# zhengchen1999/DOVE

Measured on AMD Instinct MI355X. Metric: SR frames/s (33x720x1280 4x one-step, whole job), higher is better.
Workload: dtype bf16; 1 GPU; synthetic 33x720x1280 HR clip (LR 180x320, 4x), one-step t=399, CogVideoX1.5-5B VAE + 42-layer DiT random-init, 1 clip per GPU (BASELINE configs[1]); weight_sums=True, vae_streams=2, variant=headline (bf16)

## Files before the change

dove_amd/csrc/igemm.hip:

```cpp
#include "igemm_args.h"


template <int BN, int BK>
struct FastCfg {
  static constexpr int BM = 128;
  static constexpr int CPR = BK / 8;
  static constexpr int CPR_LOG = (BK == 64) ? 3 : 2;
  static constexpr int RPG = 256 / CPR;
  static constexpr int NA = BM / RPG;
  static constexpr int B_SLOTS = BN * CPR;
  static constexpr int NB = (B_SLOTS + 255) / 256;
  static constexpr int A_BYTES = BM * BK * 2, B_BYTES = BN * BK * 2, STAGE = A_BYTES + B_BYTES;
  static constexpr int WN = (BN >= 128) ? 2 : 1, WM = 4 / WN;
  static constexpr int PT = (BM / WM) / 32, CT = (BN / WN) / 32;
  static constexpr int KK = BK / 16;
};

template <int BN, int BK>
__global__ __launch_bounds__(256) void igemm_fast_kernel(const IgemmArgs a) {
  using Cf = FastCfg<BN, BK>;
  constexpr int NA = Cf::NA, NB = Cf::NB, PT = Cf::PT, CT = Cf::CT, KK = Cf::KK, STAGE = Cf::STAGE, A_BYTES = Cf::A_BYTES;
  extern __shared__ __attribute__((aligned(16))) char smem[];
  const int tid = threadIdx.x, lane = tid & 63;
  const int wave = __builtin_amdgcn_readfirstlane(tid >> 6);
  __builtin_assume(wave >= 0 && wave < 4);
  const int wm = wave / Cf::WN, wn = wave % Cf::WN;

  unsigned rest = xcd_remap(blockIdx.x, gridDim.x);
  const int tn = rest % a.tiles_n; rest /= a.tiles_n;
  const int twi = rest % a.tiles_w; rest /= a.tiles_w;
  const int thi = rest % a.tiles_h;
  const int t = rest / a.tiles_h;
  const int n0 = tn * BN;
  const int TWm = (1 << a.tw_log2) - 1;
  const int oh0 = thi * (128 >> a.tw_log2), ow0 = twi << a.tw_log2;

  const int cs = tid & (Cf::CPR - 1);
  const int rsub = tid >> Cf::CPR_LOG;
  const int c = (BK == 64) ? (cs ^ ((rsub >> 1) & 7)) : (cs ^ ((rsub >> 2) & 3));
  int rowoff[NA];
  unsigned mask[NA];
#pragma unroll
  for (int j = 0; j < NA; ++j) {
    const int m = j * Cf::RPG + rsub;
    const int oh = oh0 + (m >> a.tw_log2), ow = ow0 + (m & TWm);
    const bool mv = (oh < a.H_out) && (ow < a.W_out);
    const int ih0 = oh * a.stride - a.pad_h, iw0 = ow * a.stride - a.pad_w;
    rowoff[j] = ((ih0 * a.W_in + iw0) * a.Cin + c * 8) * 2;
    unsigned mk = 0;
    for (int dh = 0; dh < a.kh; ++dh)
      for (int dw = 0; dw < a.kw; ++dw) {
        const bool ok = mv && ((unsigned)(ih0 + dh) < (unsigned)a.H_in) && ((unsigned)(iw0 + dw) < (unsigned)a.W_in);
        mk |= (ok ? 1u : 0u) << (dh * a.kw + dw);
      }
    mask[j] = mk;
  }
  int boff_g[NB];
#pragma unroll
  for (int j = 0; j < NB; ++j) boff_g[j] = ((j * Cf::RPG + rsub) * a.Cin + c * 8) * 2;

  const long long frame_elems = (long long)a.H_in * a.W_in * a.Cin;
  const unsigned frame_bytes = (unsigned)(frame_elems * 2);
  const unsigned wtap_bytes = (unsigned)((long long)BN * a.Cin * 2);
  const long long wtap_stride = (long long)a.Cout_pad * a.Cin;
  const int kc_per_tap = a.Cin / BK;
  const int nk = a.kt * a.kh * a.kw * kc_per_tap;

  auto frame_ptr = [&](int dt) -> const bf16_t* { return igemm_src_frame(a, t, dt, frame_elems); };
  int s_kc = 0, s_dw = 0, s_dh = 0, s_dt = 0;
  const bf16_t* s_fp = frame_ptr(0);
  const bf16_t* s_wp = a.w + (long long)n0 * a.Cin;
  int s_tapdelta = 0;
  unsigned s_tapbit = 1u;

  auto stage = [&](auto bufc) {
// ... 1037 lines not shown
  const bool pointwise = d->kt == 1 && d->kh == 1 && d->kw == 1 && d->stride == 1 && d->up == 0 && d->tmode == 0 && d->t_in == d->t_out &&
                         d->h_in == d->h_out && d->w_in == d->w_out;
  if (pointwise && d->cin == 32 && d->act == 0 && !d->resid && !d->gate && d->cout_store >= 128) return K_SMALLK;
  if (plain_gemm) {
    if (d->cout_pad % 256 == 0 && d->cout_store % 256 == 0 && d->cin % 128 == 0 && d->cin >= 256 && (long long)256 * d->cin * 2 < (1ll << 31) &&
        d->ldo < (1 << 20) && d->ldr < (1 << 20) && (d->act == 0 || d->act == 1))
      return K_GEMM8P;
  }
  const bool conv3 = d->kh == 3 && d->kw == 3 && d->stride == 1 && d->pad_h == 1 && d->pad_w == 1 && d->act == 0 && !d->gate &&
                     d->cout_pad % 128 == 0 && frame_fits;
  if (conv3) {
    const bool same = d->up == 0 && d->tmode == 0 && d->h_out == d->h_in && d->w_out == d->w_in && d->w_out >= 16 && d->h_out >= 16;
    const bool ups = d->up == 1 && d->kt == 1 && d->h_out == 2 * d->h_in && d->w_out == 2 * d->w_in && d->h_out >= 16 && d->w_out >= 32;
    const bool h4 = d->cout_store % 128 == 0 && d->cin % 64 == 0 && d->ldo < (1 << 20) && (!d->resid || d->ldr < (1 << 20));
    if (same && h4) return K_HALO4X;
    if (ups && h4 && d->w_sub && d->h_in >= 16 && d->w_in >= 32) return K_HALO4X_SUB;
    if (ups && h4) return K_HALO4X_UP;
  }
  const int BN = (d->cout_pad % 128 == 0) ? 128 : ((d->cout_pad % 64 == 0) ? 64 : 32);
  const bool fits = frame_fits && (long long)BN * d->cin * 2 < (1ll << 31);
  return (d->up == 0 && fits) ? K_IGEMM_FAST : K_IGEMM;
}

static bool desc_size_ok(const dove_conv_desc* d, const char* who) {
  if (d && d->struct_size == sizeof(dove_conv_desc) && d->reserved == 0) return true;
  if (d) dove_set_error("%s: dove_conv_desc.struct_size is %u, this library (ABI %d) expects %zu - the caller's binding was written "
                        "against another include/dove_hip.h", who, d->struct_size, DOVE_ABI_VERSION, sizeof(dove_conv_desc));
  else dove_set_error("%s: null descriptor", who);
  return false;
}
extern "C" const char* dove_conv_kernel_name(const dove_conv_desc* d) { return desc_size_ok(d, "conv_kernel_name") ? kKernelNames[select_kernel(d)] : ""; }

template <int BN, int BK>
static int launch_igemm_fast(const IgemmArgs& a, unsigned grid, hipStream_t s) {
  constexpr int lds = 2 * (128 * BK * 2 + BN * BK * 2);
  static PerDeviceOnce attr_set;
  if (auto once_ = attr_set.guard()) (void)hipFuncSetAttribute((const void*)igemm_fast_kernel<BN, BK>, hipFuncAttributeMaxDynamicSharedMemorySize, lds);
  hipLaunchKernelGGL((igemm_fast_kernel<BN, BK>), dim3(grid), dim3(256), lds, s, a);
  DOVE_CHECK_LAUNCH("dove_conv_igemm_bf16");
  return DOVE_OK;
}

static int cu_count() {
  static std::atomic<int> cus[DOVE_MAX_DEVICES] = {};
  int dev = 0;
  (void)hipGetDevice(&dev);
  int n = (dev >= 0 && dev < DOVE_MAX_DEVICES) ? cus[dev].load(std::memory_order_relaxed) : 0;
  if (!n) {
    n = 256;
    (void)hipDeviceGetAttribute(&n, hipDeviceAttributeMultiprocessorCount, dev);
    if (dev >= 0 && dev < DOVE_MAX_DEVICES) cus[dev].store(n, std::memory_order_relaxed);
  }
  return n;
}

extern "C" long long dove_conv_gn_partial_rows(const dove_conv_desc* d) {
  if (!desc_size_ok(d, "conv_gn_partial_rows")) return 0;
  const ConvKernel k = select_kernel(d);
  if (k != K_HALO4X && k != K_HALO4X_UP && k != K_HALO4X_SUB) return 0;
  if (d->cout_store != 128 && d->cout_store != 256 && d->cout_store != 512) return 0;
  if (d->cout_store != d->cout_pad) return 0;
  if (k == K_HALO4X_SUB) {
    const long long th = (d->h_in + halo8::TH - 1) / halo8::TH, tw = (d->w_in + halo8::TW - 1) / halo8::TW;
    return (long long)desc_nb(d) * d->t_out * th * tw * 16;
  }
  const long long th = (d->h_out + halo8::TH - 1) / halo8::TH, tw = (d->w_out + halo8::TW - 1) / halo8::TW;
  return (long long)desc_nb(d) * d->t_out * th * tw * 4;
}

static bool halo4x_plan(const dove_conv_desc* d) {
  const int tiles_w = (d->w_out + halo8::TW - 1) / halo8::TW, tiles_h = (d->h_out + halo8::TH - 1) / halo8::TH;
  const int wrem = d->w_out % halo8::TW;
  if (wrem < 1 || wrem > halo8::TW / 2) return false;
  const int cus = cu_count();
  const long long per = (long long)desc_nb(d) * d->t_out * (d->cout_pad / 128);
  auto rounds = [&](long long tiles) { return (tiles * per + cus - 1) / cus; };
  return rounds((long long)tiles_h * (tiles_w - 1)) + rounds((d->h_out + 31) / 32) < rounds((long long)tiles_h * tiles_w);
}
extern "C" int dove_conv_partial_launches(const dove_conv_desc* d) {
  if (!desc_size_ok(d, "conv_partial_launches") || select_kernel(d) != K_HALO4X) return 0;
  return halo4x_plan(d) ? 1 : 0;
}

static int conv_dispatch(const dove_conv_desc* d, void* stream, ConvKernel kern);

static bool gemm_tail_split(const dove_conv_desc* d, long long* rows_main) {
  const long long M = (long long)d->t_out * d->h_out * d->w_out;
  if (d->t_out != 1 || d->h_out != 1 || desc_nb(d) > 1) return false;
  const int cus = cu_count(), tiles_n = d->cout_pad / 256;
  const long long row_tiles = (M + gemm4x::BM - 1) / gemm4x::BM, ntiles = row_tiles * tiles_n;
  if (ntiles <= cus || ntiles % cus == 0) return false;
  const long long main_rt = (ntiles / cus) * cus / tiles_n;
  if (main_rt < 1 || main_rt >= row_tiles) return false;
  const long long tail_rows = M - main_rt * gemm4x::BM;
  const long long tail_blocks = ((tail_rows + 127) / 128) * (d->cout_pad / 128);
  if (tail_blocks > 2ll * cus) return false;
  if ((long long)128 * d->cin * 2 >= (1ll << 31)) return false;
  *rows_main = main_rt * gemm4x::BM;
  return true;
}

extern "C" int dove_conv_igemm_bf16(const dove_conv_desc* d, void* stream) {
  if (!desc_size_ok(d, "conv_igemm")) return DOVE_EINVAL;
  DOVE_CHECK_ARG(d->x && d->w && d->out, "conv_igemm: null pointer");
  DOVE_CHECK_ARG(d->cin % 32 == 0 && d->cin > 0, "conv_igemm: Cin (%d) must be a positive multiple of 32 (pad on pack)", d->cin);
  DOVE_CHECK_ARG(d->cout_pad % 32 == 0 && d->cout_pad > 0, "conv_igemm: Cout_pad (%d) must be a multiple of 32", d->cout_pad);
// ... 113 lines not shown
      a.cpg_log = d->cout_store == 128 ? 2 : (d->cout_store == 256 ? 3 : 4);
      a.tiles_w = (d->w_out + halo8::TW - 1) / halo8::TW;
      a.tiles_h = (d->h_out + halo8::TH - 1) / halo8::TH;
      a.tiles_n = d->cout_pad / 128;
      a.ty0 = a.tx0 = 0; a.nty = a.tiles_h; a.ntx = a.tiles_w; a.h_lim = d->h_out; a.w_lim = d->w_out;
      const long long g4 = (long long)a.T_out * a.tiles_h * a.tiles_w * a.tiles_n;
      DOVE_CHECK_ARG(g4 > 0 && g4 < (1ll << 31), "conv_igemm: grid too large");
      static PerDeviceOnce attr4;
      if (auto once_ = attr4.guard()) {
        (void)hipFuncSetAttribute((const void*)(conv3x3_halo4x_kernel<false>), hipFuncAttributeMaxDynamicSharedMemorySize, Halo4xCfg::LDS_BYTES);
        (void)hipFuncSetAttribute((const void*)(conv3x3_halo4x_kernel<false, false, 1>), hipFuncAttributeMaxDynamicSharedMemorySize, H4Geo<1>::LDS_BYTES);
        (void)hipFuncSetAttribute((const void*)(conv3x3_halo4x_kernel<true>), hipFuncAttributeMaxDynamicSharedMemorySize, Halo4xCfg::LDS_BYTES);
      }
      const int cus = cu_count();
      const unsigned grid = g4 > cus ? (unsigned)cus : (unsigned)g4;
      if (kern == K_HALO4X_UP) hipLaunchKernelGGL((conv3x3_halo4x_kernel<true>), dim3(grid), dim3(256), Halo4xCfg::LDS_BYTES, s, a);
      else {
        const bool wpart = halo4x_plan(d);
        const int wm = wpart ? (a.tiles_w - 1) * halo8::TW : d->w_out, cols_main = wpart ? a.tiles_w - 1 : a.tiles_w;
        auto launch = [&](int part, int nty, int tx0, int ntx, int w_lim) {
          if (nty <= 0 || ntx <= 0) return;
          IgemmArgs b = a;
          b.ty0 = 0; b.nty = nty; b.tx0 = tx0; b.ntx = ntx; b.h_lim = d->h_out; b.w_lim = w_lim;
          const long long g = (long long)b.T_out * nty * ntx * b.tiles_n;
          const unsigned gr = g > cus ? (unsigned)cus : (unsigned)g;
          if (part == 0) hipLaunchKernelGGL((conv3x3_halo4x_kernel<false, false, 0>), dim3(gr), dim3(256), H4Geo<0>::LDS_BYTES, s, b);
          else hipLaunchKernelGGL((conv3x3_halo4x_kernel<false, false, 1>), dim3(gr), dim3(256), H4Geo<1>::LDS_BYTES, s, b);
        };
        launch(0, a.tiles_h, 0, cols_main, wm);
        if (wpart) launch(1, (d->h_out + 31) / 32, cols_main, 1, d->w_out);
      }
      DOVE_CHECK_LAUNCH("dove_conv_igemm_bf16(halo4x)");
      return DOVE_OK;
    }
    default: break;
  }
  int twl = 7;
  if (d->h_out > 1) {
    twl = 4;
    if (d->w_out <= 8) twl = 3;
    if (d->w_out <= 4) twl = 2;
  }
  a.tw_log2 = twl;
  const int TW = 1 << twl, TH = 128 >> twl;
  a.tiles_w = (d->w_out + TW - 1) / TW;
  a.tiles_h = (d->h_out + TH - 1) / TH;
  const int BN = (d->cout_pad % 128 == 0) ? 128 : ((d->cout_pad % 64 == 0) ? 64 : 32);
  a.tiles_n = d->cout_pad / BN;
  const long long grid = (long long)a.T_out * a.tiles_h * a.tiles_w * a.tiles_n;
  DOVE_CHECK_ARG(grid > 0 && grid < (1ll << 31), "conv_igemm: grid too large");
  const bool fast = kern == K_IGEMM_FAST;
  const bool bk64 = (d->cin % 64 == 0);
  if (!fast) return launch_igemm_legacy(a, (unsigned)grid, BN, bk64, s);
  if (BN == 128) return bk64 ? launch_igemm_fast<128, 64>(a, (unsigned)grid, s) : launch_igemm_fast<128, 32>(a, (unsigned)grid, s);
  if (BN == 64) return bk64 ? launch_igemm_fast<64, 64>(a, (unsigned)grid, s) : launch_igemm_fast<64, 32>(a, (unsigned)grid, s);
  return bk64 ? launch_igemm_fast<32, 64>(a, (unsigned)grid, s) : launch_igemm_fast<32, 32>(a, (unsigned)grid, s);
}
```

dove_amd/lib.py:

```python
from __future__ import annotations

import ctypes as C
import os

import torch

_HERE = os.path.dirname(os.path.abspath(__file__))
LIB_PATH = os.path.join(_HERE, "libdove_hip.so")
_lib = None

F32, BF16, U8 = 0, 1, 2
METRIC_PSNR, METRIC_SSIM, METRIC_RGB_TO_Y = 1, 2, 4
COLORFIX_WAVELET, COLORFIX_ADAIN, COLORFIX_CLAMP = 1, 2, 1
YUV_444, YUV_422, YUV_420, YUV_MONO = 0, 1, 2, 3
YUV_SITING_LEFT, YUV_SITING_CENTRE = 0, 1
VIDEO_RGB_U8, VIDEO_YUV = 0, 1
RESIZE_BILINEAR, RESIZE_BICUBIC, RESIZE_AREA = 0, 1, 2
ACT_NONE, ACT_RELU, ACT_SIGMOID, ACT_TANH = 0, 1, 2, 3


class ConvDesc(C.Structure):
    _fields_ = [
        ("struct_size", C.c_uint), ("reserved", C.c_uint),
        ("x", C.c_void_p), ("cache", C.c_void_p), ("w", C.c_void_p), ("bias", C.c_void_p),
# ... 186 lines not shown
    "dove_vcodec_roundtrip_tools": [_VP, _I, _I, _I, _LL, _I, _I, _VP, C.c_size_t, _VP, _VP, _VP, _VP],
    "dove_motion_search_u8": [_VP, _VP, _I, _I, _I, _I, _I, _VP, _VP, _VP],
    "dove_stitch": [_VP, _I, _I, _I, _PI, _VP, _I, _I, _I, _I, _I, _I, _VP],
    "dove_video_open": [_VP, C.POINTER(VideoParams), C.POINTER(_VP)],
    "dove_video_info": [_VP, C.POINTER(C.c_size_t), C.POINTER(C.c_size_t), _PI, _PI, _PI],
    "dove_video_push": [_VP, _VP, _I, _VP],
    "dove_video_end_of_input": [_VP],
    "dove_video_need": [_VP, _PLL, _PI],
    "dove_video_step": [_VP, _VP, C.c_size_t, _PI, _PI, _VP],
    "dove_conv2d_f32": [C.POINTER(Conv2dF32Args), _VP],
    "dove_instance_norm_f32": [_VP, _I, _I, _I, _I, _VP, _I, _F, _VP, C.c_size_t, _VP, _VP],
    "dove_corr_volume_f32": [_VP, _VP, _I, _I, _I, _I, _F, _VP, _VP],
    "dove_avgpool2_f32": [_VP, _LL, _I, _I, _VP, _VP],
    "dove_corr_lookup_f32": [_VP, _VP, _VP, _VP, _VP, _LL, _I, _I, _I, _I, _VP, _VP],
    "dove_gru_gate_f32": [_VP, _LL, _VP, _LL, _I, _I, _LL, _VP, _VP],
    "dove_gru_update_f32": [_VP, _LL, _VP, _LL, _VP, _LL, _I, _LL, _VP],
    "dove_add_f32": [_VP, _LL, _VP, _LL, _VP, _LL, _I, _LL, _I, _VP],
    "dove_convex_upsample_f32": [_VP, _LL, _VP, _I, _I, _I, _VP, _VP],
    "dove_flow_warp_error": [_VP, _VP, _I, _VP, _VP, _I, _I, _I, _VP, C.c_size_t, _VP, _VP, _VP, _VP],
    "dove_convnet_conv_f32": [C.POINTER(ConvnetConvF32Args), _VP],
    "dove_percep_prep_f32": [C.POINTER(ImageView), _I, _I, _I, _I, _F, _F, C.POINTER(C.c_float), C.POINTER(C.c_float), _VP, _VP],
    "dove_maxpool_f32": [_VP, _LL, _I, _I, _I, _I, _I, _I, _VP, _LL, _VP],
    "dove_l2pool_f32": [_VP, _LL, _I, _I, _I, _I, _VP, _LL, _VP],
    "dove_lpips_layer": [_VP, _VP, _LL, _VP, _I, _I, _I, _I, _VP, C.c_size_t, _VP, _VP],
    "dove_dists_layer": [_VP, _VP, _LL, _VP, _VP, _I, _I, _I, _I, _VP, C.c_size_t, _VP, _VP],
    "dove_niqe_features": [C.POINTER(ImageView), _I, _I, _I, _I, _VP, C.c_size_t, _VP, _VP, _VP],
    "dove_niqe_stats": [_VP, _I, _I, _VP, _VP, _VP, _VP],
    "dove_niqe_distance": [_VP, _VP, _VP, _VP, _VP],
    "dove_resnet_conv_f32": [C.POINTER(ResnetConvF32Args), _VP],
    "dove_avgpool_cl_f32": [_VP, _LL, _I, _I, _I, _I, _VP, _LL, _VP],
    "dove_clip_attnpool_f32": [_VP, _LL, _I, _I, _I, _VP, _VP, _VP, _VP, _VP, _VP, _VP, _VP, _VP, C.c_size_t, _VP, _VP],
    "dove_clipiqa_score": [_VP, _VP, _I, _I, _I, C.c_double, _VP, _VP],
    "dove_musiq_patches_f32": [C.POINTER(ImageView), _I, _I, _I, _I, C.POINTER(MusiqScale), _VP, _I, _I, _I, _VP, _VP],
    "dove_musiq_groupnorm_f32": [_VP, _VP, _VP, _VP, _VP, _VP, _LL, _I, _I, C.c_double, _I, _I, _VP, _VP],
    "dove_layernorm_f32": [_VP, _LL, _LL, _I, _VP, _VP, C.c_double, _VP, _LL, _VP],
    "dove_musiq_embed_f32": [_VP, _VP, _VP, _VP, _VP, _I, _I, _I, _VP, _VP],
    "dove_mha_f32": [_VP, _VP, _VP, _LL, _I, _I, _I, _F, _VP, _LL, _VP],
    "dove_gelu_f32": [_VP, _LL, _VP, _VP],
    "dove_musiq_score": [_VP, _LL, _VP, _VP, _I, _I, _I, _VP, _VP],
    "dove_vqa_fragments_f32": [C.POINTER(ImageView), _I, _I, _I, _VP, _I, _VP, _I, _I, _I, _I, _I, C.POINTER(C.c_double), C.POINTER(C.c_double),
                               _I, _VP, _VP],
    "dove_swin3d_window_gather_f32": [_VP, _I, _PI, _I, _PI, _PI, _VP, _VP],
    "dove_swin3d_window_scatter_f32": [_VP, _VP, _I, _PI, _I, _PI, _PI, _VP, _VP],
    "dove_swin3d_patch_merge_f32": [_VP, _LL, _I, _I, _I, _VP, _VP],
    "dove_swin3d_window_attention_f32": [_VP, _VP, _VP, _LL, _LL, _I, _I, _F, _VP, _VP, _I, _VP, _VP, _VP, _I, _VP, _LL, _VP],
    "dove_vqa_head_f64": [_VP, _LL, _I, _I, _I, _VP, _VP, _I, _VP, _VP, _VP, _VP],
    "dove_png_encode": [C.POINTER(ImageView), _I, _I, _I, _I, _VP, C.c_size_t, _VP, _VP, _VP],
    "dove_zlib_huffman": [_VP, _LL, _LL, _VP, C.c_size_t, _VP, _VP, _VP],
}
PLAIN = {"dove_last_error": (C.c_char_p, []), "dove_abi_version": (C.c_int, []), "dove_comm_destroy": (None, [C.c_void_p]),
         "dove_conv_gn_partial_rows": (C.c_longlong, [C.POINTER(ConvDesc)]),
         "dove_conv_kernel_name": (C.c_char_p, [C.POINTER(ConvDesc)]),
         "dove_conv_partial_launches": (C.c_int, [C.POINTER(ConvDesc)]),
         "dove_attention_head_paths": (C.c_int, [C.POINTER(C.c_float), _I, C.POINTER(C.c_int)]),
         "dove_attention_path_name": (C.c_char_p, [_I]),
         "dove_device_info": (C.c_int, [_I, C.c_char_p, _I, C.POINTER(C.c_int), C.POINTER(C.c_longlong)]),
         "dove_destroy": (None, [_VP]),
         "dove_vae_decode_num_frames": (C.c_int, [_VP, _I]),
         "dove_get_option": (C.c_longlong, [_VP, _I]),
         "dove_comm_useful_ranks": (C.c_int, [_VP, _I, _I]),
         "dove_workspace_bytes": (C.c_size_t, [_VP, _I, _I, _I]),
         "dove_workspace_high_water": (C.c_size_t, [_VP]),
         "dove_fr_metrics_workspace_bytes": (C.c_size_t, [_I, _I, _I]),
         "dove_color_fix_workspace_bytes": (C.c_size_t, [_I, _I, _I, _I]),
         "dove_yuv_frame_bytes": (C.c_size_t, [_I, _I, _I]),
         "dove_poisson_noise_workspace_bytes": (C.c_size_t, [_I]),
         "dove_jpeg_roundtrip_workspace_bytes": (C.c_size_t, [_I, _I, _I]),
         "dove_vcodec_workspace_bytes": (C.c_size_t, [_I, _I, _I, _I]),
         "dove_vcodec_tools_workspace_bytes": (C.c_size_t, [_I, _I, _I, _I, _I]),
         "dove_chunk_planner_need": (C.c_longlong, [_VP]),
         "dove_chunk_planner_destroy": (None, [_VP]),
         "dove_video_workspace_bytes": (C.c_size_t, [_VP, C.POINTER(VideoParams)]),
         "dove_video_close": (None, [_VP]),
         "dove_instance_norm_f32_workspace_bytes": (C.c_size_t, [_I, _I, _I, _I]),
         "dove_flow_warp_error_workspace_bytes": (C.c_size_t, [_I, _I, _I]),
         "dove_convnet_conv_f32_kernel_name": (C.c_char_p, [C.POINTER(ConvnetConvF32Args)]),
         "dove_lpips_layer_workspace_bytes": (C.c_size_t, [_I, _I, _I]),
         "dove_dists_layer_workspace_bytes": (C.c_size_t, [_I, _I, _I, _I]),
         "dove_niqe_workspace_bytes": (C.c_size_t, [_I, _I, _I]),
         "dove_resnet_conv_f32_kernel_name": (C.c_char_p, [C.POINTER(ResnetConvF32Args)]),
         "dove_clip_attnpool_workspace_bytes": (C.c_size_t, [_I, _I, _I]),
         "dove_mha_f32_tiles": (None, [C.POINTER(C.c_int), C.POINTER(C.c_int)]),
         "dove_swin3d_attention_tiles": (None, [C.POINTER(C.c_int), C.POINTER(C.c_int), C.POINTER(C.c_int)]),
         "dove_png_segment_rows": (C.c_int, [_I, _I]),
         "dove_png_bound": (C.c_size_t, [_I, _I, _I]),
         "dove_png_workspace_bytes": (C.c_size_t, [_I, _I, _I, _I]),
         "dove_zlib_huffman_bound": (C.c_size_t, [_LL, _LL]),
         "dove_zlib_huffman_workspace_bytes": (C.c_size_t, [_LL, _LL])}


def kernel_source_sha256() -> str:
    import glob
    import hashlib
    h = hashlib.sha256()
    files = sorted(glob.glob(os.path.join(_HERE, "csrc", "*.hip")) + glob.glob(os.path.join(_HERE, "csrc", "*.h")))
    files.append(os.path.join(os.path.dirname(_HERE), "include", "dove_hip.h"))
    for fn in files:
        h.update(os.path.basename(fn).encode() + b"\0")
        with open(fn, "rb") as f:
            h.update(f.read())
        h.update(b"\0")
    return h.hexdigest()


def load():
    global _lib
# ... 53 lines not shown
```

dove_amd/ops.py:

```python
from __future__ import annotations

import ctypes as C
import math
from dataclasses import dataclass

import torch

from . import lib as L


def _ru(x: int, m: int) -> int:
    return (x + m - 1) // m * m


@dataclass
class PackedConv:
    w: torch.Tensor
    bias: torch.Tensor | None
    kt: int
    kh: int
    kw: int
    cin: int
    cin_pad: int
    cout: int
# ... 24 lines not shown
        bp[:cout] = bias.detach().to(device=device, dtype=torch.float32)
    wp = wp.contiguous()
    w_first = None
    if kt == 3:
        t = wp.float().view(3, kh * kw, cout_pad, cin_pad)
        s01 = t[0] + t[1]
        w_first = torch.stack([s01, s01 + t[2]]).to(torch.bfloat16).contiguous()
    w_pair = None
    if kt == 3 and pair:
        t = wp.float().view(3, kh * kw, cout_pad, cin_pad)
        w_pair = torch.stack([t[0] + t[1], t[1] + t[2]]).to(torch.bfloat16).contiguous()
    w_sub = None
    if kt == 1 and kh == 3 and kw == 3 and sub:
        t = wp.float().view(3, 3, cout_pad, cin_pad)
        w_sub = torch.zeros(4, 4, cout_pad, cin_pad, dtype=torch.float32, device=device)
        for py in range(2):
            for px in range(2):
                for dh in range(3):
                    for dw in range(3):
                        a, b = (py + dh + 1) // 2 - py, (px + dw + 1) // 2 - px
                        w_sub[2 * py + px, 2 * a + b] += t[dh, dw]
        w_sub = w_sub.to(torch.bfloat16).contiguous()
    return PackedConv(wp, bp, kt, kh, kw, cin, cin_pad, cout, cout_pad, w_first, w_sub, w_pair)


def temporal_split(tl: int, tdup: int, cached: bool, first_sums: bool = True):
    plain = [("w0", tl - 2), ("w1", tl - 1), ("w2", tl)]
    if tdup == 0:
        if cached or not first_sums or tl > 1:
            return plain
        return [("w012", 0)] if tl == 0 else [("w01", 0), ("w2", 1)]
    if tdup == 1:
        if not cached and tl < 2:
            return [("w012", tl)]
        return [("w0", tl - 2), ("w12", tl)] if tl & 1 else [("w01", tl - 1), ("w2", tl)]
    if tl == 0:
        return [("w012", 0)]
    return [("w01", tl - 1), ("w2", tl)] if tl & 1 else [("w0", tl - 2), ("w12", tl)]


def temporal_groups(tl: int, tdup: int, cached: bool) -> int:
    return len(temporal_split(tl, tdup, cached))


_profiler = None


def set_profiler(records: list | None):
    global _profiler
    _profiler = records


def conv_kernel_name(x_shape, pc: PackedConv, *, stride=1, pad=(None, None), up=0, tmode=0, t_out=None, hw_out=None, act=0, gated=False,
                     resid=False, nb=1, partial=False):
    T, H, W, Cx = x_shape
    d = L.ConvDesc()
    d.nb = nb
    ph = (pc.kh - 1) // 2 if pad[0] is None else pad[0]
    pw = (pc.kw - 1) // 2 if pad[1] is None else pad[1]
    t_out = T if t_out is None else t_out
    if hw_out is None:
        hw_out = (H << up, W << up) if stride == 1 else ((H + 1 - pc.kh) // stride + 1, (W + 1 - pc.kw) // stride + 1)
    d.t_in, d.h_in, d.w_in, d.cin = T, H, W, Cx
    d.t_out, d.h_out, d.w_out = t_out, hw_out[0], hw_out[1]
    d.cout_pad, d.cout_store = pc.cout_pad, pc.cout_store
    d.kt, d.kh, d.kw, d.stride, d.pad_h, d.pad_w = pc.kt, pc.kh, pc.kw, stride, ph, pw
    d.up, d.tmode, d.act = up, tmode, act
    d.ldo = pc.cout_store
    d.ldr = pc.cout_store if resid else 0
    d.resid = 1 if (resid or gated) else None
    d.w_sub = 1 if (up == 1 and pc.kt == 1 and pc.kh == 3 and pc.kw == 3) else None
    d.gate = 1 if gated else None
    if partial:
        return int(L.load().dove_conv_partial_launches(C.byref(d)))
    return L.load().dove_conv_kernel_name(C.byref(d)).decode()


def conv(x: torch.Tensor, pc: PackedConv, *, cache: torch.Tensor | None = None, stride: int = 1, pad=(None, None),
         up: int = 0, tmode: int = 0, t_out: int | None = None, hw_out=None, resid: torch.Tensor | None = None,
         gate: torch.Tensor | None = None, gate_split: int = 0, act: int = 0, ldo: int | None = None,
         out: torch.Tensor | None = None,
         gn_eps: float | None = None, out_f32: bool = False, nb: int = 1, tdup: int = 0, weight_sums: bool = True) -> torch.Tensor:
    L.require_cuda(x, resid, gate, out)
    assert x.dtype == torch.bfloat16 and x.dim() == 4, (x.dtype, x.shape)
    T, H, W, Cx = x.shape
    assert T % nb == 0, (T, nb)
    T //= nb
    if Cx != pc.cin_pad:
        raise RuntimeError(f"conv: input has {Cx} channels, packed weight expects {pc.cin_pad}")
    ph = (pc.kh - 1) // 2 if pad[0] is None else pad[0]
    pw = (pc.kw - 1) // 2 if pad[1] is None else pad[1]
    if t_out is None:
        t_out = T
    if hw_out is None:
        hw_out = (H << up, W << up) if stride == 1 else ((H + 1 - pc.kh) // stride + 1, (W + 1 - pc.kw) // stride + 1)
    if ldo is None:
        ldo = pc.cout_store
    odt = torch.float32 if out_f32 else torch.bfloat16
    if out is None:
        out = torch.empty(nb * t_out, hw_out[0], hw_out[1], ldo, dtype=odt, device=x.device)
    else:
        assert out.shape == (nb * t_out, hw_out[0], hw_out[1], ldo) and out.dtype == odt
    cache_stride = 0
    if cache is not None:
        if nb > 1:
            assert cache.shape == (nb, pc.kt - 1, H, W, Cx) and cache.dtype == torch.bfloat16 and cache.is_cuda, (cache.shape, x.shape)
            assert cache[0].is_contiguous() and cache.device == x.device
            cache_stride = cache.stride(0)
        else:
            L.require_cuda(cache)
            assert cache.shape == (pc.kt - 1, H, W, Cx) and cache.dtype == torch.bfloat16, (cache.shape, x.shape)
    d = L.ConvDesc()
    d.nb, d.cache_stride = nb, cache_stride
    if cache is None and pc.w_first is not None and weight_sums:
        d.w_first = pc.w_first.data_ptr()
    if up == 1 and pc.w_sub is not None and weight_sums:
        d.w_sub = pc.w_sub.data_ptr()
    if tdup and weight_sums and pc.w_pair is not None and pc.kt == 3 and not (tdup == 2 and cache is not None):
        d.tdup, d.w_pair = tdup, pc.w_pair.data_ptr()
    d.x, d.cache, d.w = x.data_ptr(), (cache.data_ptr() if cache is not None else None), pc.w.data_ptr()
    d.bias = pc.bias.data_ptr() if pc.bias is not None else None
    d.resid = resid.data_ptr() if resid is not None else None
    d.gate = gate.data_ptr() if gate is not None else None
    d.out = out.data_ptr()
    d.t_in, d.h_in, d.w_in, d.cin = T, H, W, Cx
    d.t_out, d.h_out, d.w_out = t_out, hw_out[0], hw_out[1]
    d.cout_pad, d.cout_store = pc.cout_pad, pc.cout_store
# ... 1353 lines not shown
```

include/dove_hip.h:

```cpp
#ifndef DOVE_HIP_H
#define DOVE_HIP_H

#include <stddef.h>

#ifdef __cplusplus
extern "C" {
#endif

#define DOVE_ABI_VERSION 15

#define DOVE_F32 0
#define DOVE_BF16 1

const char* dove_last_error(void);
int dove_abi_version(void);
int dove_device_info(int dev, char* name, int name_len, int* cu_count, long long* total_mem);

typedef struct dove_conv_desc {
  unsigned int struct_size;
  unsigned int reserved;
  const void* x;
  const void* cache;
  const void* w;
  const float* bias;
  const void* resid;
  const float* gate;
  void* out;
  int t_in, h_in, w_in, cin;
  int t_out, h_out, w_out, cout_pad, cout_store;
  int kt, kh, kw, stride, pad_h, pad_w, up, tmode, act;
  long long ldo, ldr, gate_split;
  float* gn_partial;
  int out_f32;
  int nb;
  long long cache_stride;
  const void* w_first;
  const void* w_sub;
  const void* w_pair;
  int tdup;
  int reserved2;
} dove_conv_desc;
int dove_conv_igemm_bf16(const dove_conv_desc* d, void* stream);
const char* dove_conv_kernel_name(const dove_conv_desc* d);
int dove_conv_partial_launches(const dove_conv_desc* d);
long long dove_conv_gn_partial_rows(const dove_conv_desc* d);
int dove_groupnorm_finalize_partials(const float* partial, long long rows, double count, float eps, void* ws, float* stats,
                                     void* stream);

int dove_groupnorm_stats_bf16(const void* x, long long npix, long long frame_pix, int C, float eps, void* partial_ws, int ws_blocks,
                              float* stats, void* stream);
int dove_groupnorm_sums_bf16(const void* x, long long npix, long long frame_pix, int C, void* partial_ws, int ws_blocks, double* sums,
                             void* stream);
int dove_groupnorm_finalize_sums(const double* sums, double count, float eps, float* stats, void* stream);
int dove_groupnorm_sums_from_partials(const float* partial, long long rows, void* ws, double* sums, void* stream);
int dove_groupnorm_apply_bf16(const void* x, void* y, int T, int H, int W, int C, const float* stats,
                              const float* gamma, const float* beta, int silu, const void* yb, int hz, int wz,
                              int sshift, const int* tmap, void* stream);

int dove_groupnorm_stats_nb_bf16(const void* x, int nb, long long npix, long long frame_pix, int C, float eps, void* partial_ws,
                                 int ws_blocks, float* stats, void* stream);
int dove_groupnorm_finalize_partials_nb(const float* partial, long long rows, int nb, double count, float eps, void* ws, size_t ws_bytes,
                                        float* stats, void* stream);
int dove_groupnorm_apply_nb_bf16(const void* x, void* y, int nb, int T, int H, int W, int C, const float* stats, const float* gamma,
                                 const float* beta, int silu, const void* yb, int Tz, int hz, int wz, int sshift, const int* tmap,
                                 void* stream);
int dove_avgpool_time_nb_bf16(const void* x, int nb, int T, long long frame_elems, void* y, void* stream);

int dove_layernorm_modulate_bf16(const void* x, void* y, long long rows, int D, float eps, const float* gamma,
                                 const float* beta, const float* mod, long long split, void* stream);

int dove_qkv_post_bf16(const void* qkv, long long N, long long Npad, int heads, int head_dim, int text_len,
                       const float* gq, const float* bq, const float* gk, const float* bk, const float* cosT,
                       const float* sinT, float qscale, float eps, void* Qh, void* Kh, void* Vt, int v_order, float* norm2, void* stream);
int dove_vt_quad_swap_bf16(void* Vt, long long rows, long long Npad, void* stream);
int dove_ulysses_place_bf16(const void* rq, const void* rk, const void* rv, const long long* counts, int world, int hloc, long long N,
                            long long Npad, void* Qh, void* Kh, void* Vt, float* norm2_out, void* stream);

int dove_attention_fwd_bf16(const void* Qh, const void* Kh, const void* Vt, void* O, long long N, long long Npad,
                            int heads, int head_dim, long long ldo, float* norm2, void* stream);
int dove_attention_head_paths(const float* norm2_host, int heads, int* path);
const char* dove_attention_path_name(int path);

int dove_cl_from_ncthw(const void* x, int dtype, int C, long long npix, int Cp, float scale, float shift, void* y,
                       void* stream);
int dove_ncthw_from_cl(const void* x, long long ld, int C, long long npix, float scale, float shift, float lo,
                       float hi, void* y, int dtype, void* stream);
int dove_cl_im2col3x3_from_ncthw(const void* x, int dtype, int C, int T, int H, int W, int Cp, float scale, float shift, void* y,
                                 void* stream);
int dove_conv_out_gather(const float* p, long long ldp, int T, int H, int W, int C, const float* bias, float scale, float shift, float lo,
                         float hi, void* y, int dtype, void* stream);
int dove_avgpool_time_bf16(const void* x, int T, long long frame_elems, void* y, void* stream);
int dove_posterior_sample(const void* moments, long long ld, int latent_channels, long long npix, const void* noise,
                          int noise_dtype, void* out, int out_dtype, void* stream);
int dove_axpby(const void* x, const void* y, void* out, int dtype, long long n, float a, float b, void* stream);
int dove_patchify(const void* x, int dtype, int T, int C, int H, int W, int pt, int p, void* tokens, long long ld,
                  void* stream);
int dove_unpatchify(const void* tokens, long long ld, int T, int C, int H, int W, int pt, int p, void* y, int dtype,
// ... 333 lines not shown
```

Measured before the change: 35.30 frames/s.

## Add persistent weight-resident streaming path for 1x1 igemm convolutions

Adds a persistent variant of the fast igemm kernel for 1x1 (optionally kt=3) convolutions with small K. Each workgroup loads its whole weight panel into LDS once, then walks a contiguous range of 128-row tiles. Activations stream through a 3- or 6-stage LDS ring of async buffer loads, and output stores overlap with later tiles via counted vmcnt waits. The grid is sized to CUs times waves per CU, which removes repeated weight loads and per-tile launch and prologue cost. The trade-off is hand-tuned wait counts and a larger LDS footprint, and the path only applies to plain 1x1 convs with no act, resid or gate.

```diff
diff --git a/dove_amd/csrc/igemm.hip b/dove_amd/csrc/igemm.hip
--- a/dove_amd/csrc/igemm.hip
+++ b/dove_amd/csrc/igemm.hip
@@ -16,11 +16,239 @@
   static constexpr int KK = BK / 16;
 };
 
-template <int BN, int BK>
+__device__ __forceinline__ const bf16_t* fs_pin64(const bf16_t* p) {
+  const unsigned long long v = (unsigned long long)p;
+  return (const bf16_t*)(((unsigned long long)(unsigned)__builtin_amdgcn_readfirstlane((int)(v >> 32)) << 32) |
+                         (unsigned)__builtin_amdgcn_readfirstlane((int)v));
+}
+typedef __attribute__((ext_vector_type(2))) unsigned int u32x2;
+template <int N> __device__ __forceinline__ void fs_wait_vm() {
+  asm volatile("s_waitcnt vmcnt(%0)" ::"n"(N < 63 ? N : 63) : "memory");
+}
+template <int BASE, int NST> __device__ __forceinline__ void fs_wait_counted(int cnt) {
+  if (cnt == 0) fs_wait_vm<BASE>();
+  else if (cnt == 1) fs_wait_vm<BASE + NST>();
+  else if (cnt == 2) fs_wait_vm<BASE + 2 * NST>();
+  else if (cnt == 3) fs_wait_vm<BASE + 3 * NST>();
+  else if (cnt == 4) fs_wait_vm<BASE + 4 * NST>();
+  else fs_wait_vm<BASE + 5 * NST>();
+}
+
+template <int BN, int BK, int NS>
+__device__ __forceinline__ void igemm_stream_walk(const IgemmArgs& a, char* smem) {
+  using Cf = FastCfg<BN, BK>;
+  constexpr int NA = Cf::NA, NB = Cf::NB, PT = Cf::PT, CT = Cf::CT, KK = Cf::KK, A_BYTES = Cf::A_BYTES, B_BYTES = Cf::B_BYTES;
+  constexpr int AHEAD = NS - 1;
+  constexpr int NST = PT * CT * 4;
+  constexpr int RING = NS * A_BYTES;
+  static_assert(NS >= 3 && NS <= 6, "ring of 3..6 stages (fs_wait_counted counts up to 5 epilogues)");
+  const int tid = threadIdx.x, lane = tid & 63;
+  const int wave = __builtin_amdgcn_readfirstlane(tid >> 6);
+  __builtin_assume(wave >= 0 && wave < 4);
+  const int wm = wave / Cf::WN, wn = wave % Cf::WN;
+  const int hi = lane >> 5, l31 = lane & 31;
+
+  const unsigned wg = xcd_remap(blockIdx.x, gridDim.x);
+  const int tn = (int)(wg % (unsigned)a.tiles_n), rb = (int)(wg / (unsigned)a.tiles_n), GR = (int)(gridDim.x / (unsigned)a.tiles_n);
+  const long long RT = (long long)a.T_out * a.tiles_h;
+  const int tile0 = __builtin_amdgcn_readfirstlane((int)(rb * RT / GR)), tile1 = __builtin_amdgcn_readfirstlane((int)((rb + 1) * RT / GR));
+  const int n0 = tn * BN;
+  const int HW = a.H_out * a.W_out;
+  const long long frame_elems = (long long)HW * a.Cin;
+  const unsigned frame_bytes = (unsigned)(frame_elems * 2);
+  const int kc_per_tap = a.Cin / BK;
+  const int nk = a.kt * kc_per_tap;
+  const int nsteps = (tile1 - tile0) * nk;
+
+  const int cs = tid & (Cf::CPR - 1);
+  const int rsub = tid >> Cf::CPR_LOG;
+  const int c = (BK == 64) ? (cs ^ ((rsub >> 1) & 7)) : (cs ^ ((rsub >> 2) & 3));
+  unsigned rowoff[NA];
+#pragma unroll
+  for (int j = 0; j < NA; ++j) rowoff[j] = (unsigned)(((j * Cf::RPG + rsub) * a.Cin + c * 8) * 2);
+
+  f32x4 biasr[CT][4];
+#pragma unroll
+  for (int i = 0; i < CT; ++i)
+#pragma unroll
+    for (int g = 0; g < 4; ++g) {
+      const int cb = n0 + wn * (BN / Cf::WN) + i * 32 + 8 * g + 4 * hi;
+      biasr[i][g] = (a.bias && cb < a.Cout_st) ? *(const f32x4*)(a.bias + cb) : f32x4{0.f, 0.f, 0.f, 0.f};
+    }
+  __builtin_amdgcn_s_waitcnt(0x0F70);
+
+  {
+    const unsigned wtap_bytes = (unsigned)((long long)BN * a.Cin * 2);
+    const bf16_t* wp = a.w + (long long)n0 * a.Cin;
+    int ks = 0;
+    for (int tap = 0; tap < a.kt; ++tap, wp += (long long)a.Cout_pad * a.Cin) {
+      const auto srd_b = __builtin_amdgcn_make_buffer_rsrc((void*)wp, (short)0, (int)wtap_bytes, 0x00020000);
+      for (int kc = 0; kc < kc_per_tap; ++kc, ++ks) {
+#pragma unroll
+        for (int j = 0; j < NB; ++j) {
+          if (j * 256 + wave * 64 < Cf::B_SLOTS)
+            __builtin_amdgcn_raw_ptr_buffer_load_lds(srd_b, (lds_ptr_t)(smem + RING + ks * B_BYTES + (j * 256 + wave * 64) * 16), 16,
+                                                     (unsigned)(((j * Cf::RPG + rsub) * a.Cin + c * 8) * 2), kc * (BK * 2), 0, 0);
+        }
+      }
+    }
+  }
+
+  int s_tile = tile0, s_t = tile0 / a.tiles_h, s_rt = tile0 - s_t * a.tiles_h, s_dt = 0, s_kc = 0;
+  const bf16_t* s_fp = a.x;
+  int s_nrec = 0;
+  auto open = [&]() {
+    const bool on = s_tile < tile1;
+    const long long roff = (long long)s_rt * 128 * a.Cin;
+    s_fp = fs_pin64(igemm_src_frame(a, on ? s_t : 0, s_dt, frame_elems) + roff);
+    s_nrec = on ? (int)(frame_bytes - (unsigned)(roff * 2)) : 0;
+  };
+  open();
+  auto stage = [&](int slot) {
+    const auto srd_a = __builtin_amdgcn_make_buffer_rsrc((void*)s_fp, (short)0, s_nrec, 0x00020000);
+    const int soff = s_kc * (BK * 2);
+#pragma unroll
+    for (int j = 0; j < NA; ++j)
+      __builtin_amdgcn_raw_ptr_buffer_load_lds(srd_a, (lds_ptr_t)(smem + slot * A_BYTES + (j * 256 + wave * 64) * 16), 16, rowoff[j], soff, 0, 0);
+    if (++s_kc == kc_per_tap) {
+      s_kc = 0;
+      if (++s_dt == a.kt) {
+        s_dt = 0;
+        ++s_tile;
+        if (++s_rt == a.tiles_h) { s_rt = 0; ++s_t; }
+      }
+      open();
+    }
+  };
+
+  int aoff[PT][KK], boff[CT][KK];
+#pragma unroll
+  for (int kk = 0; kk < KK; ++kk) {
+    const int chunk = kk * 2 + hi;
+#pragma unroll
+    for (int p = 0; p < PT; ++p) {
+      const int row = wm * (Cf::BM / Cf::WM) + p * 32 + l31;
+      const int sc = (BK == 64) ? (chunk ^ ((row >> 1) & 7)) : (chunk ^ ((row >> 2) & 3));
+      aoff[p][kk] = row * (BK * 2) + sc * 16;
+    }
+#pragma unroll
+    for (int i = 0; i < CT; ++i) {
+      const int row = wn * (BN / Cf::WN) + i * 32 + l31;
+      const int sc = (BK == 64) ? (chunk ^ ((row >> 1) & 7)) : (chunk ^ ((row >> 2) & 3));
+      boff[i][kk] = RING + row * (BK * 2) + sc * 16;
+    }
+  }
+
+  f32x16 acc[CT][PT];
+  auto zero_acc = [&]() {
+#pragma unroll
+    for (int i = 0; i < CT; ++i)
+#pragma unroll
+      for (int p = 0; p < PT; ++p)
+#pragma unroll
+        for (int r = 0; r < 16; ++r) acc[i][p][r] = 0.f;
+  };
+  zero_acc();
+
+  const int es = a.out_f32 ? 4 : 2;
+  const int ldo_b = (int)a.ldo * es;
+  unsigned ooff[PT];
+#pragma unroll
+  for (int p = 0; p < PT; ++p) ooff[p] = (unsigned)((wm * (Cf::BM / Cf::WM) + p * 32 + l31) * ldo_b);
+  auto epilogue = [&](int c_t, int c_rt, auto f32c, auto biasc) {
+    constexpr bool kF32 = decltype(f32c)::value, kBias = decltype(biasc)::value;
+    const int left = HW - c_rt * 128, rows = left < 128 ? left : 128;
+    const char* ob = (const char*)a.out + ((long long)c_t * HW + (long long)c_rt * 128) * ldo_b;
+    const auto srd_o = __builtin_amdgcn_make_buffer_rsrc((void*)fs_pin64((const bf16_t*)ob), (short)0, rows * ldo_b, 0x00020000);
+#pragma unroll
+    for (int p = 0; p < PT; ++p) {
+#pragma unroll
+      for (int i = 0; i < CT; ++i) {
+#pragma unroll
+        for (int g = 0; g < 4; ++g) {
+          const int cb = n0 + wn * (BN / Cf::WN) + i * 32 + 8 * g + 4 * hi;
+          float v[4];
+#pragma unroll
+          for (int e = 0; e < 4; ++e) v[e] = acc[i][p][g * 4 + e];
+          if (kBias) {
+#pragma unroll
+            for (int e = 0; e < 4; ++e) v[e] += biasr[i][g][e];
+          }
+          const unsigned voff = cb < a.Cout_st ? ooff[p] + (unsigned)(cb * es) : 0x80000000u;
+          if (kF32) {
+            __builtin_amdgcn_raw_buffer_store_b128(u32x4{__float_as_uint(v[0]), __float_as_uint(v[1]), __float_as_uint(v[2]), __float_as_uint(v[3])},
+                                                   srd_o, (int)voff, 0, 0);
+            __builtin_amdgcn_sched_barrier(0);
+            asm volatile("s_nop 3" ::: "memory");
+            __builtin_amdgcn_sched_barrier(0);
+          } else {
+            __builtin_amdgcn_raw_buffer_store_b64(u32x2{pack_bf2(v[0], v[1]), pack_bf2(v[2], v[3])}, srd_o, (int)voff, 0, 0);
+          }
+        }
+      }
+    }
+    __builtin_amdgcn_sched_barrier(0);
+    asm volatile("s_nop 3" ::: "memory");
+    __builtin_amdgcn_sched_barrier(0);
+  };
+
+#pragma unroll
+  for (int u = 0; u < AHEAD; ++u) stage(u);
+
+  int c_t = tile0 / a.tiles_h, c_rt = tile0 - c_t * a.tiles_h, c_k = 0;
+  int slot = 0, nslot = AHEAD;
+  unsigned hist = 0;
+  for (int s = 0; s < nsteps; ++s) {
+    fs_wait_counted<(AHEAD - 1) * NA, NST>(__builtin_popcount(hist & ((1u << AHEAD) - 1)));
+    __builtin_amdgcn_s_barrier();
+    asm volatile("" ::: "memory");
+    stage(nslot);
+    {
+      const int sa = slot * A_BYTES, sb = c_k * B_BYTES;
+#pragma unroll
+      for (int kk = 0; kk < KK; ++kk) {
+        bf16x8 xf[PT], wf[CT];
+#pragma unroll
+        for (int p = 0; p < PT; ++p) xf[p] = *(const bf16x8*)(smem + sa + aoff[p][kk]);
+#pragma unroll
+        for (int i = 0; i < CT; ++i) wf[i] = *(const bf16x8*)(smem + sb + boff[i][kk]);
+#pragma unroll
+        for (int i = 0; i < CT; ++i)
+#pragma unroll
+          for (int p = 0; p < PT; ++p)
+            acc[i][p] = __builtin_amdgcn_mfma_f32_32x32x16_bf16(wf[i], xf[p], acc[i][p], 0, 0, 0);
+      }
+    }
+    asm volatile("" ::: "memory");
+    slot = slot + 1 == NS ? 0 : slot + 1;
+    nslot = nslot + 1 == NS ? 0 : nslot + 1;
+    hist <<= 1;
+    if (++c_k == nk) {
+      if (a.out_f32) {
+        if (a.bias) epilogue(c_t, c_rt, std::true_type{}, std::true_type{});
+        else epilogue(c_t, c_rt, std::true_type{}, std::false_type{});
+      } else {
+        if (a.bias) epilogue(c_t, c_rt, std::false_type{}, std::true_type{});
+        else epilogue(c_t, c_rt, std::false_type{}, std::false_type{});
+      }
+      zero_acc();
+      c_k = 0;
+      hist |= 1u;
+      if (++c_rt == a.tiles_h) { c_rt = 0; ++c_t; }
+    }
+  }
+  asm volatile("s_waitcnt vmcnt(0)" ::: "memory");
+}
+
+template <int BN, int BK, int kStream = 0>
 __global__ __launch_bounds__(256) void igemm_fast_kernel(const IgemmArgs a) {
   using Cf = FastCfg<BN, BK>;
   constexpr int NA = Cf::NA, NB = Cf::NB, PT = Cf::PT, CT = Cf::CT, KK = Cf::KK, STAGE = Cf::STAGE, A_BYTES = Cf::A_BYTES;
   extern __shared__ __attribute__((aligned(16))) char smem[];
+  if constexpr (kStream > 0) {
+    igemm_stream_walk<BN, BK, kStream>(a, smem);
+    return;
+  }
   const int tid = threadIdx.x, lane = tid & 63;
   const int wave = __builtin_amdgcn_readfirstlane(tid >> 6);
   __builtin_assume(wave >= 0 && wave < 4);
@@ -1164,6 +1392,46 @@
     if (dev >= 0 && dev < DOVE_MAX_DEVICES) cus[dev].store(n, std::memory_order_relaxed);
   }
   return n;
+}
+
+struct StreamPlan { int ns, wpc; };
+static StreamPlan igemm_stream_plan(const dove_conv_desc* d) {
+  const StreamPlan no{0, 0};
+  if (select_kernel(d) != K_IGEMM_FAST) return no;
+  if (d->kh != 1 || d->kw != 1 || d->stride != 1 || d->up != 0 || d->nb > 1 || (d->kt != 1 && d->kt != 3)) return no;
+  if ((long long)d->kt * d->cin > 512) return no;
+  if (d->tmode != 0 || d->pad_h != 0 || d->pad_w != 0 || d->t_in != d->t_out || d->h_in != d->h_out || d->w_in != d->w_out) return no;
+  if (d->act != 0 || d->resid || d->gate || d->ldo >= (1 << 20)) return no;
+  const int BN = (d->cout_pad % 128 == 0) ? 128 : ((d->cout_pad % 64 == 0) ? 64 : 32), BK = (d->cin % 64 == 0) ? 64 : 32;
+  const int panel = d->kt * d->cin * BN * 2, stage = 128 * BK * 2, lds_cu = 160 * 1024;
+  StreamPlan p;
+  if (panel + 6 * stage <= lds_cu / 2) p = StreamPlan{6, 2};
+  else if (panel + 6 * stage <= lds_cu) p = StreamPlan{6, 1};
+  else if (panel + 3 * stage <= lds_cu) p = StreamPlan{3, 1};
+  else return no;
+  const long long row_tiles = (long long)d->t_out * (((long long)d->h_out * d->w_out + 127) / 128);
+  if (row_tiles < 2ll * cu_count() || row_tiles >= (1ll << 31)) return no;
+  return p;
+}
+extern "C" int dove_conv_igemm_fast_streams(const dove_conv_desc* d) {
+  if (!desc_size_ok(d, "conv_igemm_fast_streams")) return 0;
+  return igemm_stream_plan(d).ns ? 1 : 0;
+}
+
+template <int BN, int BK, int NS>
+static int launch_igemm_stream(const IgemmArgs& a, unsigned grid, hipStream_t s) {
+  const int lds = NS * (128 * BK * 2) + a.kt * a.Cin * BN * 2;
+  static PerDeviceOnce attr_set;
+  if (auto once_ = attr_set.guard()) (void)hipFuncSetAttribute((const void*)igemm_fast_kernel<BN, BK, NS>, hipFuncAttributeMaxDynamicSharedMemorySize, 160 * 1024);
+  hipLaunchKernelGGL((igemm_fast_kernel<BN, BK, NS>), dim3(grid), dim3(256), lds, s, a);
+  DOVE_CHECK_LAUNCH("dove_conv_igemm_bf16(stream)");
+  return DOVE_OK;
+}
+template <int NS>
+static int launch_igemm_stream_ns(const IgemmArgs& a, unsigned grid, int BN, bool bk64, hipStream_t s) {
+  if (BN == 128) return bk64 ? launch_igemm_stream<128, 64, NS>(a, grid, s) : launch_igemm_stream<128, 32, NS>(a, grid, s);
+  if (BN == 64) return bk64 ? launch_igemm_stream<64, 64, NS>(a, grid, s) : launch_igemm_stream<64, 32, NS>(a, grid, s);
+  return bk64 ? launch_igemm_stream<32, 64, NS>(a, grid, s) : launch_igemm_stream<32, 32, NS>(a, grid, s);
 }
 
 extern "C" long long dove_conv_gn_partial_rows(const dove_conv_desc* d) {
@@ -1383,6 +1651,15 @@
   const bool fast = kern == K_IGEMM_FAST;
   const bool bk64 = (d->cin % 64 == 0);
   if (!fast) return launch_igemm_legacy(a, (unsigned)grid, BN, bk64, s);
+  if (const StreamPlan sp = igemm_stream_plan(d); sp.ns) {
+    a.tw_log2 = 7; a.tiles_w = 1;
+    a.tiles_h = (int)(((long long)d->h_out * d->w_out + 127) / 128);
+    const long long row_tiles = (long long)a.T_out * a.tiles_h;
+    long long groups = (long long)cu_count() * sp.wpc / a.tiles_n;
+    groups = groups < 1 ? 1 : (groups > row_tiles ? row_tiles : groups);
+    const unsigned g = (unsigned)(groups * a.tiles_n);
+    return sp.ns == 6 ? launch_igemm_stream_ns<6>(a, g, BN, bk64, s) : launch_igemm_stream_ns<3>(a, g, BN, bk64, s);
+  }
   if (BN == 128) return bk64 ? launch_igemm_fast<128, 64>(a, (unsigned)grid, s) : launch_igemm_fast<128, 32>(a, (unsigned)grid, s);
   if (BN == 64) return bk64 ? launch_igemm_fast<64, 64>(a, (unsigned)grid, s) : launch_igemm_fast<64, 32>(a, (unsigned)grid, s);
   return bk64 ? launch_igemm_fast<32, 64>(a, (unsigned)grid, s) : launch_igemm_fast<32, 32>(a, (unsigned)grid, s);
diff --git a/dove_amd/lib.py b/dove_amd/lib.py
--- a/dove_amd/lib.py
+++ b/dove_amd/lib.py
@@ -262,6 +262,7 @@
          "dove_conv_gn_partial_rows": (C.c_longlong, [C.POINTER(ConvDesc)]),
          "dove_conv_kernel_name": (C.c_char_p, [C.POINTER(ConvDesc)]),
          "dove_conv_partial_launches": (C.c_int, [C.POINTER(ConvDesc)]),
+         "dove_conv_igemm_fast_streams": (C.c_int, [C.POINTER(ConvDesc)]),
          "dove_attention_head_paths": (C.c_int, [C.POINTER(C.c_float), _I, C.POINTER(C.c_int)]),
          "dove_attention_path_name": (C.c_char_p, [_I]),
          "dove_device_info": (C.c_int, [_I, C.c_char_p, _I, C.POINTER(C.c_int), C.POINTER(C.c_longlong)]),
diff --git a/dove_amd/ops.py b/dove_amd/ops.py
--- a/dove_amd/ops.py
+++ b/dove_amd/ops.py
@@ -100,7 +100,7 @@
 
 
 def conv_kernel_name(x_shape, pc: PackedConv, *, stride=1, pad=(None, None), up=0, tmode=0, t_out=None, hw_out=None, act=0, gated=False,
-                     resid=False, nb=1, partial=False):
+                     resid=False, nb=1, partial=False, streams=False):
     T, H, W, Cx = x_shape
     d = L.ConvDesc()
     d.nb = nb
@@ -121,6 +121,8 @@
     d.gate = 1 if gated else None
     if partial:
         return int(L.load().dove_conv_partial_launches(C.byref(d)))
+    if streams:
+        return int(L.load().dove_conv_igemm_fast_streams(C.byref(d)))
     return L.load().dove_conv_kernel_name(C.byref(d)).decode()
 
 
diff --git a/include/dove_hip.h b/include/dove_hip.h
--- a/include/dove_hip.h
+++ b/include/dove_hip.h
@@ -43,6 +43,7 @@
 int dove_conv_igemm_bf16(const dove_conv_desc* d, void* stream);
 const char* dove_conv_kernel_name(const dove_conv_desc* d);
 int dove_conv_partial_launches(const dove_conv_desc* d);
+int dove_conv_igemm_fast_streams(const dove_conv_desc* d);
 long long dove_conv_gn_partial_rows(const dove_conv_desc* d);
 int dove_groupnorm_finalize_partials(const float* partial, long long rows, double count, float eps, void* ws, float* stats,
                                      void* stream);
```

Measured after the change: 35.44 frames/s, median of 6. About the same (+0.4%).
